# chinajuanbob/istio

Hardware: AMD Instinct MI355X
Metric: request x rule predicate evals/sec at 10k rules (higher is better)
Workload: dtype u32; 1 GPU; C2 rules scaled to R=10000, 1048576 requests per GPU (configs[1] family, configs[4] shard); rules=10000, requests_per_gpu=1048576, parallelism=request-sharded dp1

## Files before the change

istio_amd/csrc/kernels.hip:

```cpp
#include <hip/hip_runtime.h>
#include <stdint.h>
#include <type_traits>

#include "../../include/mxp_batch.h"
#include "kargs.h"
#include "pack_args.h"
#include "vm.h"

namespace {

__device__ __forceinline__ uint32_t uni(uint32_t v) { return __builtin_amdgcn_readfirstlane(v); }

typedef __attribute__((address_space(4))) const mxp_kargs ckargs;
__device__ __forceinline__ ckargs& kargs_view() {
    ckargs* p = (ckargs*)__builtin_amdgcn_kernarg_segment_ptr();
    asm volatile("" : "+s"(p));
    return *p;
}

__device__ __forceinline__ uint32_t wave_max(uint32_t v) {
#pragma unroll
    for (int off = 32; off > 0; off >>= 1) v = max(v, (uint32_t)__shfl_xor((int)v, off, 64));
    return __builtin_amdgcn_readfirstlane(v);
}
// ... 997 lines not shown
                }
                if (old == key) break;
                h = (h + 1u) & (cap - 1u);
            }
            lcls[i] = h;
            if (count) atomicAdd(A.vt_cnt + kb + h, lcnt[i]);
        }
        __syncthreads();
        (void)loc;
        __syncthreads();
    }
}

extern "C" __global__ __launch_bounds__(256) void mxp_vtd_final_kernel(mxp_kargs A, mxp_vtd_final_args F) {
    const uint32_t a = blockIdx.y, i = blockIdx.x * 256u + threadIdx.x;
    if (i >= MXP_VTD_CAP) return;
    const uint64_t at = (uint64_t)F.cand[a] * MXP_VTD_CAP + i;
    const unsigned long long key = F.tkey[at];
    if (key == MXP_VT_EMPTY) return;
    const uint32_t cap = A.vt_meta[a * 8u + MXP_VTM_CAP], kb = A.vt_meta[a * 8u + MXP_VTM_KBASE];
    unsigned long long* T = A.vt_keys + kb;
    uint32_t h = mxp_hash64(key) & (cap - 1u);
    while (atomicCAS(T + h, (unsigned long long)MXP_VT_EMPTY, key) != MXP_VT_EMPTY) h = (h + 1u) & (cap - 1u);
    const uint2 cr = F.tcr[at];
    A.vt_rep[kb + h] = cr.y;
    A.vt_cnt[kb + h] = cr.x;
}

extern "C" hipError_t mxp_launch_vtd_final(const mxp_kargs* args, const mxp_vtd_final_args* f, hipStream_t s) {
    hipLaunchKernelGGL(mxp_vtd_final_kernel, dim3(MXP_VTD_CAP / 256u, args->n_vt), dim3(256), 0, s, *args, *f);
    return hipGetLastError();
}

__device__ __forceinline__ uint32_t vt_probe(const unsigned long long* __restrict__ T, uint32_t cap,
                                             unsigned long long key) {
    uint32_t h = mxp_hash64(key) & (cap - 1u);
    for (uint32_t i = 0; i < cap; i++, h = (h + 1u) & (cap - 1u)) {
        const unsigned long long k = T[h];
        if (k == key || k == MXP_VT_EMPTY) break;
    }
    return h;
}
extern "C" __global__ __launch_bounds__(256) void mxp_vt_lookup_kernel(mxp_kargs A) {
    const uint32_t a = blockIdx.y, q = A.q0 + (blockIdx.x * 256u + threadIdx.x) * 4u, Q1 = A.q1;
    if (q >= Q1) return;
    const uint64_t N = A.n;
    const uint32_t col = uni(A.vt_meta[a * 8u + MXP_VTM_COL]), cap = uni(A.vt_meta[a * 8u + MXP_VTM_CAP]),
                   kb = uni(A.vt_meta[a * 8u + MXP_VTM_KBASE]);
    const unsigned long long* __restrict__ T = A.vt_keys + kb;
    const uint64_t at = (uint64_t)col * N + q;
    uint16_t* const C = A.vt_cls + (uint64_t)a * MXP_VT_PITCH(N) + q;
    if ((N & 3u) == 0 && (q & 3u) == 0 && q + 4u <= Q1) {
        const uint32_t k4 = *(const uint32_t*)(A.kinds + at);
        const ulonglong2 v01 = *(const ulonglong2*)(A.vals + at), v23 = *(const ulonglong2*)(A.vals + at + 2u);
        const uint32_t h0 = vt_probe(T, cap, mxp_vt_key(k4 & 0xFFu, v01.x));
        const uint32_t h1 = vt_probe(T, cap, mxp_vt_key((k4 >> 8) & 0xFFu, v01.y));
        const uint32_t h2 = vt_probe(T, cap, mxp_vt_key((k4 >> 16) & 0xFFu, v23.x));
        const uint32_t h3 = vt_probe(T, cap, mxp_vt_key(k4 >> 24, v23.y));
        *(uint64_t*)C = (uint64_t)h0 | (uint64_t)h1 << 16 | (uint64_t)h2 << 32 | (uint64_t)h3 << 48;
        return;
    }
    for (uint32_t r = 0; r < 4u && q + r < Q1; r++)
        C[r] = (uint16_t)vt_probe(T, cap, mxp_vt_key(A.kinds[at + r], A.vals[at + r]));
}

template <bool kNfa>
__device__ __forceinline__ void vt_eval_body(const mxp_kargs& A, uint64_t (*regs)[256]) {
    const uint32_t tid = threadIdx.x;
    const uint32_t lane = tid & 63u;
    const uint32_t wave = uni(tid >> 6);
    uint32_t t = blockIdx.x, a = 0;
    for (; a + 1 < A.n_vt; a++) {
        const uint32_t nt = uni(A.vt_meta[a * 8u + MXP_VTM_CAP]) / 64u;
        if (t < nt) break;
        t -= nt;
    }
    const uint32_t* M = A.vt_meta + a * 8u;
    const uint32_t cap = uni(M[MXP_VTM_CAP]), kb = uni(M[MXP_VTM_KBASE]), tb = uni(M[MXP_VTM_TBASE]),
                   nw = uni(M[MXP_VTM_NW]), woff = uni(M[MXP_VTM_WOFF]);
    const uint32_t j = blockIdx.y * 4u + wave;
    if (j >= nw || t * 64u >= cap) return;
    const uint32_t k = t * 64u + lane;
    const bool live = __hip_atomic_load(A.vt_keys + kb + k, __ATOMIC_RELAXED, __HIP_MEMORY_SCOPE_AGENT) != MXP_VT_EMPTY;
    const uint32_t rep = live ? A.vt_rep[kb + k] : 0u;
    const uint32_t g = uni(A.vt_words[2u * (woff + j)]), mask = uni(A.vt_words[2u * (woff + j) + 1u]);
    uint32_t m = 0, e = 0;
    for (uint32_t bits = mask; bits; bits &= bits - 1u) {
        const uint32_t b = __builtin_ctz(bits);
        const uint32_t rule = g * 32u + b;
        const uint32_t base = uni(A.rule_off[rule]);
        const uint32_t len = uni(A.rule_off[rule + 1]) - base;
        const uint32_t code = run_rule<false, kNfa>(A, ((cuint32*)A.prog) + (uint64_t)base * 4u, len, 0u, live, rule, rep, regs, tid);
        if (live) {
            m |= code == PC_TRUE ? 1u << b : 0u;
            e |= code >= PC_ERROR ? 1u << b : 0u;
        }
    }
    *(uint2*)(A.vt_tm + 2u * ((uint64_t)tb + (uint64_t)j * cap + k)) = make_uint2(m, e);
    if (counting(A)) {
        const uint32_t c = live ? A.vt_cnt[kb + k] : 0u;
        for (uint32_t bits = wave_or(live ? m : 0u); bits; bits &= bits - 1u) {
            const uint32_t bb = __builtin_ctz(bits);
            uint32_t sum = (m >> bb) & 1u ? c : 0u;
#pragma unroll
            for (int off = 32; off > 0; off >>= 1) sum += (uint32_t)__shfl_xor((int)sum, off, 64);
            if (lane == 0 && sum) atomicAdd(A.hits + g * 32u + bb, (unsigned long long)sum);
        }
    }
}

extern "C" __global__ __launch_bounds__(256) void mxp_vt_eval_kernel(mxp_kargs A) {
    __shared__ uint64_t regs[MXP_VM_MAXREG][256];
    vt_eval_body<false>(A, regs);
}

extern "C" __global__ __launch_bounds__(256) void mxp_vt_eval_nfa_kernel(mxp_kargs A) {
    __shared__ uint64_t regs[MXP_VM_MAXREG][256];
    vt_eval_body<true>(A, regs);
}

__device__ __forceinline__ void sort8(uint32_t (&x)[8]) {
#define MXP_CX(a, b)                          \
    {                                         \
        const uint32_t lo = min(x[a], x[b]);  \
        x[b] = max(x[a], x[b]);               \
        x[a] = lo;                            \
    }
    MXP_CX(0, 1) MXP_CX(2, 3) MXP_CX(4, 5) MXP_CX(6, 7) MXP_CX(0, 2) MXP_CX(1, 3) MXP_CX(4, 6) MXP_CX(5, 7)
    MXP_CX(1, 2) MXP_CX(5, 6) MXP_CX(0, 4) MXP_CX(1, 5) MXP_CX(2, 6) MXP_CX(3, 7) MXP_CX(2, 4) MXP_CX(3, 5)
    MXP_CX(1, 2) MXP_CX(3, 4) MXP_CX(5, 6)
#undef MXP_CX
}

__device__ __forceinline__ void dtp_merge(uint32_t x, bool on, uint32_t (&m)[4], uint32_t (&e)[4]) {
    const uint32_t b = on ? 1u << (x & 31u) : 0u, r = (x >> 5) & 3u;
    const uint32_t bm = (x & 128u) ? 0u : b, be = (x & 128u) ? b : 0u;
#pragma unroll
    for (uint32_t k = 0; k < 4; k++) {
        m[k] |= r == k ? bm : 0u;
        e[k] |= r == k ? be : 0u;
    }
}

struct DtpQueue {
    uint32_t q0 = ~0u, q1 = ~0u, q2 = ~0u, q3 = ~0u;
    __device__ __forceinline__ void load(const mxp_kargs& A, uint32_t chunk, uint32_t req0, bool in) {
        if (!A.dtp_slots || !in) return;
        typedef uint32_t v4u __attribute__((ext_vector_type(4)));
        const uint64_t qi = (uint64_t)chunk * MXP_DTP_ROW(A.dtp_tiles) + (req0 >> 2);
        const uint32_t dk = A.dtp_qn[qi];
        const v4u sl = *(const v4u*)(A.dtp_slots + qi * 8u);
        decode(dk, sl);
    }
    __device__ __forceinline__ void load_live(const uint16_t* slots, const uint8_t* qn, uint32_t tiles, uint32_t chunk,
                                              uint32_t req0, bool in) {
        if (!in) return;
        typedef uint32_t v4u __attribute__((ext_vector_type(4)));
        const uint64_t qi = (uint64_t)chunk * MXP_DTP_ROW(tiles) + (req0 >> 2);
        const uint32_t dk = qn[qi];
        if (!dk) return;
        const v4u sl = *(const v4u*)(slots + qi * 8u);
        decode(dk, sl);
    }
    __device__ __forceinline__ uint32_t head_group() const { return (q0 & 0xFFFFu) == 0xFFFFu ? 256u : (q0 >> 8) & 0xFFu; }
    __device__ __forceinline__ bool take(uint32_t g, uint32_t (&m)[4]) {
        bool named = false;
        while (head_group() == g) {
            const uint32_t x = q0 & 0xFFFFu;
            const bool mp = !(x & 128u);
            const uint32_t b = mp ? 1u << (x & 31u) : 0u, r = (x >> 5) & 3u;
#pragma unroll
            for (uint32_t k = 0; k < 4; k++) m[k] |= r == k ? b : 0u;
            named |= mp;
            q0 = __builtin_amdgcn_alignbit(q1, q0, 16);
            q1 = __builtin_amdgcn_alignbit(q2, q1, 16);
            q2 = __builtin_amdgcn_alignbit(q3, q2, 16);
            q3 = q3 >> 16 | 0xFFFF0000u;
        }
        return named;
    }
    template <typename V4>
    __device__ __forceinline__ void decode(uint32_t dk, const V4& sl) {
        if (!dk) return;
        const uint32_t h[4] = {sl.x, sl.y, sl.z, sl.w};
        uint32_t x[8];
#pragma unroll
        for (uint32_t i = 0; i < 8; i++) x[i] = i < dk ? (h[i >> 1] >> (16u * (i & 1u))) & 0xFFFFu : 0xFFFFu;
        sort8(x);
        q0 = x[0] | x[1] << 16;
        q1 = x[2] | x[3] << 16;
        q2 = x[4] | x[5] << 16;
        q3 = x[6] | x[7] << 16;
    }
    __device__ __forceinline__ bool any_err() const { return __ballot(has_err()) != 0; }
    __device__ __forceinline__ bool has_err() const {
        bool h = false;
        const uint32_t w[4] = {q0, q1, q2, q3};
#pragma unroll
        for (int i = 0; i < 8; i++) {
            const uint32_t x = (w[i >> 1] >> (16 * (i & 1))) & 0xFFFFu;
            h |= x != 0xFFFFu && (x & 128u);
        }
        return h;
    }
    template <uint32_t G, bool kErr>
    __device__ __forceinline__ void merge_c(uint32_t (&m)[4], uint32_t (&e)[4]) {
        for (;;) {
            const uint32_t x = q0;
            const bool hit = ((x >> 8) & 0xFFu) == G;
            if (!__ballot(hit)) break;
            const uint32_t b = hit ? 1u << (x & 31u) : 0u, r = (x >> 5) & 3u;
            const uint32_t bm = (kErr && (x & 128u)) ? 0u : b;
#pragma unroll
            for (uint32_t k = 0; k < 4; k++) m[k] |= r == k ? bm : 0u;
            if (kErr) {
                const uint32_t be = (x & 128u) ? b : 0u;
#pragma unroll
                for (uint32_t k = 0; k < 4; k++) e[k] |= r == k ? be : 0u;
            }
            if (hit) {
                q0 = __builtin_amdgcn_alignbit(q1, q0, 16);
                q1 = __builtin_amdgcn_alignbit(q2, q1, 16);
                q2 = __builtin_amdgcn_alignbit(q3, q2, 16);
                q3 = q3 >> 16 | 0xFFFF0000u;
            }
        }
    }
    __device__ __forceinline__ void merge(uint32_t g, uint32_t (&m)[4], uint32_t (&e)[4]) {
        for (;;) {
            const uint32_t x = q0 & 0xFFFFu;
            const bool hit = (x >> 8) == g;
            if (!__ballot(hit)) break;
            dtp_merge(x, hit, m, e);
            if (hit) {
                q0 = __builtin_amdgcn_alignbit(q1, q0, 16);
                q1 = __builtin_amdgcn_alignbit(q2, q1, 16);
                q2 = __builtin_amdgcn_alignbit(q3, q2, 16);
                q3 = q3 >> 16 | 0xFFFF0000u;
            }
        }
    }
};

template <bool kLds>
__device__ __forceinline__ void vtfill_wave(const mxp_kargs& A, const mxp_fill* F, uint32_t chunk, uint32_t qw,
                                            const uint2* S, const uint32_t* RW) {
    const uint32_t lane = threadIdx.x & 63u;
    const uint32_t col = uni(F->col), okset = uni(F->okset), g0 = uni(F->g0), n = uni(F->n), moff = uni(F->moff);
    const uint64_t N = A.n;
    const uint32_t Q1 = A.q1;
    if (qw >= Q1) return;
    const uint32_t q0 = qw + lane * 4u;
    const bool vec = (N & 3u) == 0 && (Q1 & 3u) == 0 && (q0 & 3u) == 0;
    const uint32_t nvt = uni(A.n_vt);
    uint32_t bad[4];
    typedef uint32_t vcls __attribute__((ext_vector_type(2 * MXP_VT_MAX)));
    vcls clv;
#pragma unroll
    for (int r = 0; r < 4; r++) {
        const bool in = q0 + r < Q1;
        const uint32_t k = in ? A.kinds[(uint64_t)col * N + q0 + r] : 0u;
        bad[r] = (in && !((okset >> k) & 1u)) ? ~0u : 0u;
    }
#pragma unroll
    for (uint32_t a = 0; a < MXP_VT_MAX; a++) {
        uint64_t c = 0;
        if (a < nvt) {
            const uint16_t* C = A.vt_cls + (uint64_t)a * MXP_VT_PITCH(N);
            if (vec && q0 < Q1) {
                c = *(const uint64_t*)(C + q0);
            } else {
                for (uint32_t r = 0; r < 4; r++)
                    if (q0 + r < Q1) c |= (uint64_t)C[q0 + r] << (16u * r);
            }
        }
        clv[2 * a] = (uint32_t)c;
        clv[2 * a + 1] = (uint32_t)(c >> 32);
    }
    const bool any = (bad[0] | bad[1] | bad[2] | bad[3]) != 0;
    DtpQueue dq;
    dq.load(A, chunk, q0, q0 < Q1);
    const bool dany = __ballot(dq.q0 != ~0u) != 0;
    const bool nt = !(A.flags & 128u);
    typedef uint32_t v4u __attribute__((ext_vector_type(4)));
    const uint32_t MV = lane < 2u * MXP_VT_MAX && (lane >> 1) < nvt ? A.vt_meta[(lane >> 1) * 8u + MXP_VTM_CAP + (lane & 1u)] : 0u;
    const uint32_t FM = lane < n ? A.fill_masks[moff + lane] : 0u;
    const uint32_t GM = kLds && lane < n ? A.gvt_mask[g0 + lane] : 0u;
    const uint32_t GO = lane <= n ? A.gvt_off[g0 + lane] : 0u;
    const uint32_t e0 = __builtin_amdgcn_readlane(GO, 0), ecount = __builtin_amdgcn_readlane(GO, n) - e0;
    uint32_t GE0 = lane < ecount ? A.gvt[e0 + lane] : 0u, GE1 = lane + 64u < ecount ? A.gvt[e0 + 64u + lane] : 0u;
    uint32_t anyerr[4] = {0u, 0u, 0u, 0u};
    for (uint32_t g = 0; g < n; g++) {
        const uint32_t G = g0 + g;
        const uint32_t mask = __builtin_amdgcn_readlane(FM, g);
        uint32_t m[4] = {0u, 0u, 0u, 0u}, e[4], ve[4] = {0u, 0u, 0u, 0u};
#pragma unroll
        for (int r = 0; r < 4; r++) e[r] = bad[r] & mask;
        if (A.errlog && any && mask)
            for (uint32_t r = 0; r < 4; r++)
                if (e[r] && q0 + r < Q1) log_guard_errors(A, e[r], G * 32u, q0 + r);
        const uint32_t i0 = __builtin_amdgcn_readlane(GO, g) - e0, i1 = __builtin_amdgcn_readlane(GO, g + 1) - e0;
        if constexpr (kLds) {
            const uint32_t gm = __builtin_amdgcn_readlane(GM, g);
            const uint4 ra = *(const uint4*)(RW + g * MXP_VT_MAX), rb = *(const uint4*)(RW + g * MXP_VT_MAX + 4u);
            const uint32_t rows[MXP_VT_MAX] = {ra.x, ra.y, ra.z, ra.w, rb.x, rb.y, rb.z, rb.w};
#pragma unroll
            for (uint32_t a = 0; a < MXP_VT_MAX; a++) {
                if (!(gm & (1u << a))) continue;
                const uint32_t row = rows[a];
                const uint64_t c = (uint64_t)clv[2u * a] | (uint64_t)clv[2u * a + 1u] << 32;
#pragma unroll
                for (uint32_t r = 0; r < 4; r++) {
                    const uint2 w = S[row + ((uint32_t)(c >> (16u * r)) & 0xFFFFu)];
                    m[r] |= w.x;
                    ve[r] |= w.y;
                }
            }
        } else
        for (uint32_t i = i0; i < i1; i++) {
            const uint32_t ent = i < 64u ? __builtin_amdgcn_readlane(GE0, i)
                                 : i < 128u ? __builtin_amdgcn_readlane(GE1, i - 64u) : uni(A.gvt[e0 + i]);
            const uint32_t a = ent >> 24, j = ent & 0xFFFFFFu;
            const uint32_t au = __builtin_amdgcn_readfirstlane(a);
            const uint64_t c = (uint64_t)clv[2u * au] | (uint64_t)clv[2u * au + 1u] << 32;
            if constexpr (kLds) {
                const uint32_t row = j;
#pragma unroll
                for (uint32_t r = 0; r < 4; r++) {
                    const uint2 w = S[row + ((uint32_t)(c >> (16u * r)) & 0xFFFFu)];
                    m[r] |= w.x;
                    ve[r] |= w.y;
                }
            } else {
                const uint32_t cap = __builtin_amdgcn_readlane(MV, 2u * a);
                const uint32_t tb = __builtin_amdgcn_readlane(MV, 2u * a + 1u);
                const uint64_t row = (uint64_t)tb + (uint64_t)j * cap;
#pragma unroll
                for (uint32_t r = 0; r < 4; r++) {
                    const uint2 w = *(const uint2*)(A.vt_tm + 2u * (row + ((c >> (16u * r)) & 0xFFFFu)));
                    m[r] |= w.x;
                    ve[r] |= w.y;
                }
            }
        }
        uint32_t vmask[4];
#pragma unroll
        for (int r = 0; r < 4; r++) {
            vmask[r] = q0 + r < Q1 ? ~0u : 0u;
            e[r] |= ve[r];
        }
        if (A.errlog) {
            uint32_t c = 0;
#pragma unroll
            for (int r = 0; r < 4; r++) c += (uint32_t)__builtin_popcount(ve[r] & vmask[r]);
            vt_count_n(A, c);
        }
        if (dany) dq.merge(g, m, e);
#pragma unroll
        for (uint32_t r = 0; r < 4; r++) anyerr[r] |= e[r];
        const uint64_t at = (uint64_t)G * N + q0;
        if (vec && q0 < Q1) {
            const v4u mv = v4u{m[0], m[1], m[2], m[3]};
            const v4u ev = v4u{e[0], e[1], e[2], e[3]};
            if (nt) {
                if (A.out_match) __builtin_nontemporal_store(mv, (v4u*)(A.out_match + at));
                if (A.out_err) __builtin_nontemporal_store(ev, (v4u*)(A.out_err + at));
            } else {
                if (A.out_match) *(v4u*)(A.out_match + at) = mv;
                if (A.out_err) *(v4u*)(A.out_err + at) = ev;
            }
        } else {
            for (uint32_t r = 0; r < 4; r++) {
                if (q0 + r >= Q1) break;
                if (A.out_match) A.out_match[at + r] = m[r];
                if (A.out_err) A.out_err[at + r] = e[r];
            }
        }
    }
    if (A.req_err)
        for (uint32_t r = 0; r < 4; r++)
            if (anyerr[r] && q0 + r < Q1) A.req_err[q0 + r] = 1;
}

extern "C" __global__ __launch_bounds__(256) void mxp_fill_dtp_kernel(mxp_kargs A) {
    const uint32_t lane = threadIdx.x & 63u;
    const uint32_t wave = uni(threadIdx.x >> 6);
    const mxp_fill* F = A.fills + blockIdx.y;
    const uint32_t col = uni(F->col), okset = uni(F->okset), g0 = uni(F->g0), n = uni(F->n), moff = uni(F->moff);
    const uint64_t N = A.n;
    const uint32_t Q1 = A.q1;
    const uint32_t qw = A.q0 + (blockIdx.x * 4u + wave) * 256u;
    if (qw >= Q1) return;
    const uint32_t q0 = qw + lane * 4u;
    const bool vec = (N & 3u) == 0 && (Q1 & 3u) == 0;
    uint32_t bad[4];
#pragma unroll
    for (int r = 0; r < 4; r++) {
        const bool in = q0 + r < Q1;
        const uint32_t k = in ? A.kinds[(uint64_t)col * N + q0 + r] : 0u;
        bad[r] = (in && !((okset >> k) & 1u)) ? ~0u : 0u;
    }
    const bool any = (bad[0] | bad[1] | bad[2] | bad[3]) != 0;
    const bool store = !A.dtp_lazy || uni(*A.dtp_lazy) != 0u;
    const bool sparse = A.ret_w && uni(A.ret_w[0]) == 0u;
    DtpQueue dq, dp;
    if (sparse) {
        dq.load_live(A.dtp_slots, A.dtp_qn, A.dtp_tiles, A.dtp_cbase + blockIdx.y, q0, q0 < Q1);
        dp.load_live(A.dtp_pslots, A.dtp_pqn, A.dtp_tiles, A.dtp_cbase + blockIdx.y, q0, q0 < Q1);
    } else if (store) {
        dq.load(A, A.dtp_cbase + blockIdx.y, q0, q0 < Q1);
    }
    const bool dany = __ballot(dq.q0 != ~0u) != 0;
    if (A.req_err && any) {
        uint32_t masks = 0;
        for (uint32_t g = 0; g < n; g++) masks |= uni(A.fill_masks[moff + g]);
        if (masks)
            for (uint32_t r = 0; r < 4; r++)
                if (bad[r] && q0 + r < Q1) A.req_err[q0 + r] = 1;
    }
    if (A.errlog && any)
        for (uint32_t g = 0; g < n; g++) {
            const uint32_t mask = uni(A.fill_masks[moff + g]);
            for (uint32_t r = 0; r < 4; r++)
                if (bad[r] && q0 + r < Q1) log_guard_errors(A, mask, (g0 + g) * 32u, q0 + r);
        }
    if (!store) return;
    const bool nt = !(A.flags & 128u);
    typedef uint32_t v4u __attribute__((ext_vector_type(4)));
    if (sparse) {
        const bool snt = (A.flags & 4194304u) != 0u;
        for (;;) {
            const uint32_t g = min(dq.head_group(), dp.head_group());
            if (g >= n) break;
            uint32_t m[4] = {0u, 0u, 0u, 0u}, z[4] = {0u, 0u, 0u, 0u};
            const bool cur = dq.take(g, m);
            const bool was = dp.take(g, z);
            if (cur || was) {
                const uint64_t at = (uint64_t)(g0 + g) * N + q0;
                if (vec) {
                    const v4u mv = v4u{m[0], m[1], m[2], m[3]};
                    if (snt)
                        __builtin_nontemporal_store(mv, (v4u*)(A.out_match + at));
                    else
                        *(v4u*)(A.out_match + at) = mv;
                } else {
                    for (uint32_t r = 0; r < 4; r++)
                        if (q0 + r < Q1) A.out_match[at + r] = m[r];
                }
            }
        }
        return;
    }
    for (uint32_t g = 0; g < n; g++) {
        const uint32_t mask = uni(A.fill_masks[moff + g]);
        uint32_t m[4] = {0u, 0u, 0u, 0u}, e[4];
#pragma unroll
        for (int r = 0; r < 4; r++) e[r] = bad[r] & mask;
        if (dany) dq.merge(g, m, e);
        const uint64_t at = (uint64_t)(g0 + g) * N + q0;
        if (vec && q0 < Q1) {
            const v4u mv = v4u{m[0], m[1], m[2], m[3]}, ev = v4u{e[0], e[1], e[2], e[3]};
            if (nt) {
                if (A.out_match) __builtin_nontemporal_store(mv, (v4u*)(A.out_match + at));
                if (A.out_err) __builtin_nontemporal_store(ev, (v4u*)(A.out_err + at));
            } else {
                if (A.out_match) *(v4u*)(A.out_match + at) = mv;
                if (A.out_err) *(v4u*)(A.out_err + at) = ev;
            }
        } else {
            for (uint32_t r = 0; r < 4; r++) {
                if (q0 + r >= Q1) break;
                if (A.out_match) A.out_match[at + r] = m[r];
                if (A.out_err) A.out_err[at + r] = e[r];
            }
        }
    }
}

extern "C" __global__ __launch_bounds__(256) void mxp_vtfill_kernel(mxp_kargs A) {
    const uint32_t wave = uni(threadIdx.x >> 6);
    vtfill_wave<false>(A, A.fills + blockIdx.y, A.dtp_cbase + blockIdx.y, A.q0 + (blockIdx.x * 4u + wave) * 256u, nullptr,
                       nullptr);
}

#define MXP_VTF_STAGE 4096u
extern "C" __global__ __launch_bounds__(256) void mxp_vtfill_lds_kernel(mxp_kargs A) {
    __shared__ uint2 S[MXP_VTF_STAGE];
    const uint32_t tid = threadIdx.x, lane = tid & 63u, wave = uni(tid >> 6);
    const mxp_fill* F = A.fills + blockIdx.y;
    const uint32_t g0 = uni(F->g0), n = uni(F->n), nvt = uni(A.n_vt);
    const uint32_t e0 = uni(A.gvt_off[g0]), ecount = uni(A.gvt_off[g0 + n]) - e0;
    const uint32_t E0 = lane < ecount ? A.gvt[e0 + lane] : 0xFFFFFFFFu;
    const uint32_t E1 = lane + 64u < ecount ? A.gvt[e0 + 64u + lane] : 0xFFFFFFFFu;
    const uint32_t capl = lane < nvt ? A.vt_meta[lane * 8u + MXP_VTM_CAP] : 0u;
    const uint32_t tbl = lane < nvt ? A.vt_meta[lane * 8u + MXP_VTM_TBASE] : 0u;
    uint32_t PB = 0, PJ = 0, total = 0;
    for (uint32_t a = 0; a < nvt; a++) {
        const uint32_t lo = wave_min(min((E0 >> 24) == a ? (E0 & 0xFFFFFFu) : 0xFFFFFFFFu,
                                         (E1 >> 24) == a ? (E1 & 0xFFFFFFu) : 0xFFFFFFFFu));
        const uint32_t hi = wave_max(max((E0 >> 24) == a && E0 != 0xFFFFFFFFu ? (E0 & 0xFFFFFFu) + 1u : 0u,
                                         (E1 >> 24) == a && E1 != 0xFFFFFFFFu ? (E1 & 0xFFFFFFu) + 1u : 0u));
        const uint32_t rows = hi > lo ? hi - lo : 0u;
        if (lane == a) {
            PB = total;
            PJ = rows ? lo : 0u;
        }
        total += rows * __builtin_amdgcn_readlane(capl, a);
    }
    const bool staged = ecount <= 128u && n <= MXP_FILL_CHUNK && total <= MXP_VTF_STAGE && !(A.flags & 2097152u);
    __shared__ uint32_t RW[MXP_FILL_CHUNK * MXP_VT_MAX];
    __shared__ uint32_t PL[3 * MXP_VT_MAX];
    if (staged) {
        for (uint32_t a = 0; a < nvt; a++) {
            const uint32_t base = __builtin_amdgcn_readlane(PB, a);
            const uint32_t next = a + 1u < nvt ? __builtin_amdgcn_readlane(PB, a + 1u) : total;
            const uint64_t src = (uint64_t)__builtin_amdgcn_readlane(tbl, a) +
                                 (uint64_t)__builtin_amdgcn_readlane(PJ, a) * __builtin_amdgcn_readlane(capl, a);
            for (uint32_t i = tid; i < next - base; i += 256u) S[base + i] = *(const uint2*)(A.vt_tm + 2u * (src + i));
        }
        if (tid < nvt) {
            PL[3u * tid] = PB;
            PL[3u * tid + 1u] = PJ;
            PL[3u * tid + 2u] = capl;
        }
        __syncthreads();
        if (tid < n) {
            const uint32_t i1 = A.gvt_off[g0 + tid + 1u];
            for (uint32_t i = A.gvt_off[g0 + tid]; i < i1; i++) {
                const uint32_t ent = A.gvt[i], a = ent >> 24, j = ent & 0xFFFFFFu;
                RW[tid * MXP_VT_MAX + a] = PL[3u * a] + (j - PL[3u * a + 1u]) * PL[3u * a + 2u];
            }
        }
        __syncthreads();
    }
    for (uint32_t t = 0; t < MXP_VTF_TILES; t++) {
        const uint32_t qw = A.q0 + ((blockIdx.x * MXP_VTF_TILES + t) * 4u + wave) * 256u;
        if (staged)
            vtfill_wave<true>(A, F, A.dtp_cbase + blockIdx.y, qw, S, RW);
        else
            vtfill_wave<false>(A, F, A.dtp_cbase + blockIdx.y, qw, nullptr, nullptr);
    }
}

#define MXP_VTI_CAP 64u
template <uint32_t V>
struct GroupC {
    static constexpr uint32_t value = V;
    static constexpr bool ct = true;
};
struct GroupR {
    uint32_t value;
    static constexpr bool ct = false;
};
template <uint32_t G, uint32_t NG, typename F>
__device__ __forceinline__ void for_groups(F& f) {
    if constexpr (G < NG) {
        f(GroupC<G>{});
        for_groups<G + 1, NG>(f);
    }
}
template <uint32_t NVT, bool kSlow>
__device__ __forceinline__ void vtfill_imm_body(const mxp_kargs& A, uint32_t bx, uint32_t by, uint32_t gx) {
    __shared__ uint32_t SM[NVT * MXP_FILL_CHUNK * MXP_VTI_CAP];
    __shared__ uint32_t SJ[NVT * MXP_FILL_CHUNK];
    __shared__ uint32_t eflag;
    const uint32_t tid = threadIdx.x, lane = tid & 63u, wave = uni(tid >> 6);
    uint8_t* const slow = A.vtf_slow + ((uint64_t)by * gx + bx) * (MXP_VTF_TILES * 4u);
    if constexpr (kSlow) {
        if (!__syncthreads_or(tid < MXP_VTF_TILES * 4u ? slow[tid] : 0)) return;
    }
    const mxp_fill* F = A.fills + by;
    const uint32_t col = uni(F->col), okset = uni(F->okset), g0 = uni(F->g0), n = uni(F->n), moff = uni(F->moff);
    const uint32_t chunk = A.dtp_cbase + by;
    for (uint32_t i = tid; i < NVT * MXP_FILL_CHUNK * MXP_VTI_CAP; i += 256u) SM[i] = 0u;
    if (tid < NVT * MXP_FILL_CHUNK) SJ[tid] = ~0u;
    if (tid == 0) eflag = 0u;
    __syncthreads();
    const uint32_t TB = lane < NVT ? A.vt_meta[lane * 8u + MXP_VTM_TBASE] : 0u;
    uint32_t eor = 0u;
    for (uint32_t g = 0; g < n; g++) {
        const uint32_t i0 = uni(A.gvt_off[g0 + g]), i1 = uni(A.gvt_off[g0 + g + 1u]);
        for (uint32_t x = tid; x < (i1 - i0) * MXP_VTI_CAP; x += 256u) {
            const uint32_t ent = A.gvt[i0 + x / MXP_VTI_CAP], a = ent >> 24, j = ent & 0xFFFFFFu, k = x % MXP_VTI_CAP;
            const uint32_t tb = __builtin_amdgcn_ds_bpermute((int)(a << 2), (int)TB);
            const uint2 w = *(const uint2*)(A.vt_tm + 2u * ((uint64_t)tb + (uint64_t)j * MXP_VTI_CAP + k));
            SM[(a * MXP_FILL_CHUNK + g) * MXP_VTI_CAP + k] = w.x;
            if (k == 0) SJ[a * MXP_FILL_CHUNK + g] = j;
            eor |= w.y;
        }
    }
    if (__ballot(eor != 0u)) {
        if (lane == 0) atomicOr(&eflag, 1u);
    }
    __syncthreads();
    const bool errs = eflag != 0u;
    const uint64_t N = A.n;
    const uint32_t Q1 = A.q1;
    const bool nt = !(A.flags & 128u);
    typedef uint32_t v4u __attribute__((ext_vector_type(4)));
    const uint32_t FM = lane < n ? A.fill_masks[moff + lane] : 0u;
    struct TileIn {
        uint32_t k4, dk;
        uint64_t c[NVT];
        v4u sl;
    };
    auto fetch = [&](uint32_t t, TileIn& T) __attribute__((always_inline)) {
        const uint32_t q0 = A.q0 + ((bx * MXP_VTF_TILES + t) * 4u + wave) * 256u + lane * 4u;
        const bool vec = (N & 3u) == 0 && (Q1 & 3u) == 0 && (q0 & 3u) == 0;
        T.k4 = 0u;
        if (vec && q0 < Q1) {
            T.k4 = *(const uint32_t*)(A.kinds + (uint64_t)col * N + q0);
        } else {
            for (uint32_t r = 0; r < 4; r++)
                if (q0 + r < Q1) T.k4 |= (uint32_t)A.kinds[(uint64_t)col * N + q0 + r] << (8u * r);
        }
#pragma unroll
        for (uint32_t a = 0; a < NVT; a++) {
            const uint16_t* C = A.vt_cls + (uint64_t)a * MXP_VT_PITCH(N);
            uint64_t c = 0;
            if (vec && q0 < Q1) {
                c = *(const uint64_t*)(C + q0);
            } else {
                for (uint32_t r = 0; r < 4; r++)
                    if (q0 + r < Q1) c |= (uint64_t)C[q0 + r] << (16u * r);
            }
            T.c[a] = c;
        }
        T.dk = 0u;
// ... 896 lines not shown
        if (bits && A.out_match) atomicOr(A.out_match + (uint64_t)w * A.n + req, bits);
        t += (uint32_t)__builtin_popcount(bits);
    }
    if (A.stats) {
#pragma unroll
        for (int off = 32; off > 0; off >>= 1) t += (uint32_t)__shfl_xor((int)t, off, 64);
        if (lane == 0 && t) atomicAdd((unsigned long long*)A.stats, (unsigned long long)t);
    }
}

namespace {

__device__ __forceinline__ void csa(uint32_t& h, uint32_t& l, uint32_t a, uint32_t b, uint32_t c) {
    const uint32_t u = a ^ b;
    h = (a & b) | (u & c);
    l = u ^ c;
}

__device__ __forceinline__ uint32_t hs16(const uint32_t* d, uint32_t& ones, uint32_t& twos, uint32_t& fours,
                                         uint32_t& eights) {
    uint32_t twosA, twosB, foursA, foursB, eightsA, eightsB, sixteens;
    csa(twosA, ones, ones, d[0], d[1]);
    csa(twosB, ones, ones, d[2], d[3]);
    csa(foursA, twos, twos, twosA, twosB);
    csa(twosA, ones, ones, d[4], d[5]);
    csa(twosB, ones, ones, d[6], d[7]);
    csa(foursB, twos, twos, twosA, twosB);
    csa(eightsA, fours, fours, foursA, foursB);
    csa(twosA, ones, ones, d[8], d[9]);
    csa(twosB, ones, ones, d[10], d[11]);
    csa(foursA, twos, twos, twosA, twosB);
    csa(twosA, ones, ones, d[12], d[13]);
    csa(twosB, ones, ones, d[14], d[15]);
    csa(foursB, twos, twos, twosA, twosB);
    csa(eightsB, fours, fours, foursA, foursB);
    csa(sixteens, eights, eights, eightsA, eightsB);
    return sixteens;
}

template <bool kVec>
__device__ __forceinline__ void hits_body(const uint32_t* __restrict__ row, uint32_t n, uint32_t n_rules,
                                          unsigned long long* __restrict__ hits) {
    const uint32_t w = blockIdx.x;
    const uint32_t nthreads = gridDim.y * blockDim.x;
    const uint32_t t = blockIdx.y * blockDim.x + threadIdx.x;
    uint32_t ones = 0, twos = 0, fours = 0, eights = 0, sixteens = 0;
    uint32_t P[8];
#pragma unroll
    for (int j = 0; j < 8; j++) P[j] = 0;
    for (uint64_t base = 0; base < n; base += nthreads * 32u) {
        uint32_t d[32];
        if (kVec) {
#pragma unroll
            for (int j = 0; j < 8; j++) {
                const uint64_t i = base + ((uint64_t)j * nthreads + t) * 4u;
                uint4 v = make_uint4(0, 0, 0, 0);
                if (i < n) v = *(const uint4*)(row + i);
                d[4 * j] = v.x;
                d[4 * j + 1] = v.y;
                d[4 * j + 2] = v.z;
                d[4 * j + 3] = v.w;
            }
        } else {
#pragma unroll
            for (int j = 0; j < 32; j++) {
                const uint64_t i = base + (uint64_t)j * nthreads + t;
                d[j] = i < n ? row[i] : 0u;
            }
        }
        const uint32_t sA = hs16(d, ones, twos, fours, eights);
        const uint32_t sB = hs16(d + 16, ones, twos, fours, eights);
        uint32_t thirtytwos;
        csa(thirtytwos, sixteens, sixteens, sA, sB);
#pragma unroll
        for (int j = 0; j < 8; j++) P[j] += (thirtytwos >> j) & 0x01010101u;
    }
    __shared__ uint32_t red[32][8];
#pragma unroll
    for (int k = 0; k < 32; k++) {
        uint32_t c = 32u * ((P[k & 7] >> (8 * (k >> 3))) & 0xFFu) + 16u * ((sixteens >> k) & 1u) +
                     8u * ((eights >> k) & 1u) + 4u * ((fours >> k) & 1u) + 2u * ((twos >> k) & 1u) + ((ones >> k) & 1u);
        for (int off = 32; off > 0; off >>= 1) c += __shfl_xor((int)c, off, 64);
        if ((threadIdx.x & 63) == 0) red[k][threadIdx.x >> 6] = c;
    }
    __syncthreads();
    if (threadIdx.x < 32) {
        uint32_t c = 0;
        for (uint32_t i = 0; i < blockDim.x / 64; i++) c += red[threadIdx.x][i];
        const uint32_t rule = w * 32 + threadIdx.x;
        if (rule < n_rules && c) atomicAdd(&hits[rule], (unsigned long long)c);
    }
}

}

__device__ __forceinline__ void next_gate(unsigned long long* stats, uint32_t* gate_next, uint32_t n, uint32_t force) {
    if (!gate_next || blockIdx.x || blockIdx.y || threadIdx.x) return;
    const unsigned long long v = *stats;
    *gate_next = force == 1u ? 1u : force == 2u ? 0u : (v * 125ull <= (unsigned long long)gridDim.x * n ? 1u : 0u);
    *stats = 0ull;
}

extern "C" __global__ __launch_bounds__(256) void mxp_hits_kernel(const uint32_t* __restrict__ match, uint32_t n,
                                                                  uint32_t n_rules,
                                                                  unsigned long long* __restrict__ hits,
                                                                  const uint32_t* __restrict__ gate,
                                                                  unsigned long long* stats, uint32_t* gate_next,
                                                                  uint32_t force) {
    next_gate(stats, gate_next, n, force);
    if (gate && *gate) return;
    hits_body<true>(match + (uint64_t)blockIdx.x * n, n, n_rules, hits);
}

extern "C" __global__ __launch_bounds__(256) void mxp_hits_ragged_kernel(const uint32_t* __restrict__ match, uint32_t n,
                                                                         uint32_t n_rules,
                                                                         unsigned long long* __restrict__ hits,
                                                                         const uint32_t* __restrict__ gate,
                                                                         unsigned long long* stats, uint32_t* gate_next,
                                                                         uint32_t force) {
    next_gate(stats, gate_next, n, force);
    if (gate && *gate) return;
    hits_body<false>(match + (uint64_t)blockIdx.x * n, n, n_rules, hits);
}

extern "C" hipError_t mxp_launch_eval(const mxp_kargs* args, uint32_t grid_x, uint32_t grid_y, int vm, hipStream_t s) {
    if (vm == 2 && args->refs)
        hipLaunchKernelGGL(mxp_eval_deep_refs_kernel, dim3(grid_x, grid_y), dim3(256), 0, s, *args);
    else if (vm == 2 && args->nfa)
        hipLaunchKernelGGL(mxp_eval_deep_nfa_kernel, dim3(grid_x, grid_y), dim3(256), 0, s, *args);
    else if (vm == 2)
        hipLaunchKernelGGL(mxp_eval_deep_kernel, dim3(grid_x, grid_y), dim3(256), 0, s, *args);
    else if (vm && args->refs)
        hipLaunchKernelGGL(mxp_eval_refs_kernel, dim3(grid_x, grid_y), dim3(256), 0, s, *args);
    else if (vm && args->nfa)
        hipLaunchKernelGGL(mxp_eval_nfa_kernel, dim3(grid_x, grid_y), dim3(256), 0, s, *args);
    else if (vm)
        hipLaunchKernelGGL(mxp_eval_kernel, dim3(grid_x, grid_y), dim3(256), 0, s, *args);
    else if (args->flags & 65536u)
        hipLaunchKernelGGL(mxp_guard_kernel, dim3(grid_x, grid_y), dim3(256), 0, s, *args);
    else
        hipLaunchKernelGGL(mxp_guard2_kernel, dim3((grid_x + 1) / 2, grid_y), dim3(256), 0, s, *args);
    return hipGetLastError();
}

extern "C" hipError_t mxp_launch_dtp_hits(const uint32_t* part, uint32_t tiles, uint32_t n_rules,
                                          unsigned long long* hits, hipStream_t s) {
    const uint32_t R2 = (n_rules + 1u) / 2u;
    hipLaunchKernelGGL(mxp_dtp_hits_kernel, dim3((R2 + 255u) / 256u, (tiles + 63u) / 64u), dim3(256), 0, s, part, tiles,
                       n_rules, hits);
    return hipGetLastError();
}

extern "C" hipError_t mxp_launch_fill(const mxp_kargs* args, uint32_t n_fills, hipStream_t s) {
    if (args->dtp_slots) {
        hipLaunchKernelGGL(mxp_fill_dtp_kernel, dim3((args->q1 - args->q0 + 1023u) / 1024u, n_fills), dim3(256), 0, s, *args);
        return hipGetLastError();
    }
    const uint32_t per_block = 1024u * (args->fill_span ? args->fill_span : 1u);
    hipLaunchKernelGGL(mxp_fill_kernel, dim3((args->q1 - args->q0 + per_block - 1) / per_block, n_fills), dim3(256), 0, s, *args);
    return hipGetLastError();
}

extern "C" hipError_t mxp_launch_vtfill(const mxp_kargs* args, uint32_t n_fills, hipStream_t s) {
    if (args->flags & 2097152u) {
        hipLaunchKernelGGL(mxp_vtfill_kernel, dim3((args->q1 - args->q0 + 1023u) / 1024u, n_fills), dim3(256), 0, s, *args);
    } else {
        const uint32_t per = 1024u * MXP_VTF_TILES;
        const dim3 grid((args->q1 - args->q0 + per - 1u) / per, n_fills);
        void (*k)(mxp_kargs) = mxp_vtfill_lds_kernel;
        void (*ks)(mxp_kargs, uint32_t, uint32_t) = nullptr;
        if (args->vt_imm && args->vtf_slow && !(args->flags & 33554432u)) {
            switch (args->n_vt) {
#define MXP_VTFILL_CASE(K)                  \
    case K:                                 \
        k = mxp_vtfill_imm##K##_kernel;      \
        ks = mxp_vtfill_imm_slow##K##_kernel; \
        break;
                MXP_VTFILL_CASE(1)
                MXP_VTFILL_CASE(2)
                MXP_VTFILL_CASE(3)
                MXP_VTFILL_CASE(4)
                MXP_VTFILL_CASE(5)
                MXP_VTFILL_CASE(6)
                MXP_VTFILL_CASE(7)
                MXP_VTFILL_CASE(8)
#undef MXP_VTFILL_CASE
            default: break;
            }
        }
        hipLaunchKernelGGL(k, grid, dim3(256), 0, s, *args);
        if (ks) hipLaunchKernelGGL(ks, dim3((grid.x * grid.y + 15u) / 16u), dim3(256), 0, s, *args, grid.x, grid.y);
    }
    return hipGetLastError();
}

extern "C" hipError_t mxp_launch_dtp_sort(const mxp_kargs* args, hipStream_t s) {
    const size_t lds = args->dtp_part ? (size_t)((args->n_rules + 1u) / 2u) * 4u : 0u;
    hipLaunchKernelGGL(mxp_dtp_sort_kernel, dim3(args->dtp_tn ? args->dtp_tn : args->dtp_tiles), dim3(256), lds, s, *args);
    return hipGetLastError();
}

extern "C" hipError_t mxp_launch_vt_classify(const mxp_kargs* args, hipStream_t s) {
    hipLaunchKernelGGL(mxp_vt_classify_kernel, dim3((args->q1 - args->q0 + MXP_VTC_REQ - 1u) / MXP_VTC_REQ), dim3(256), 0, s,
                       *args);
    return hipGetLastError();
}

extern "C" hipError_t mxp_launch_vt_lookup(const mxp_kargs* args, hipStream_t s) {
    hipLaunchKernelGGL(mxp_vt_lookup_kernel, dim3((args->q1 - args->q0 + 1023u) / 1024u, args->n_vt), dim3(256), 0, s, *args);
    return hipGetLastError();
}

extern "C" hipError_t mxp_launch_vt_eval(const mxp_kargs* args, uint32_t tiles, uint32_t wchunks, hipStream_t s) {
    if (!tiles || !wchunks) return hipSuccess;
    if (args->nfa)
        hipLaunchKernelGGL(mxp_vt_eval_nfa_kernel, dim3(tiles, wchunks), dim3(256), 0, s, *args);
    else
        hipLaunchKernelGGL(mxp_vt_eval_kernel, dim3(tiles, wchunks), dim3(256), 0, s, *args);
    return hipGetLastError();
}

extern "C" hipError_t mxp_launch_inject(const mxp_kargs* args, uint32_t grid, hipStream_t s) {
    hipLaunchKernelGGL(mxp_inject_kernel, dim3(grid), dim3(256), 0, s, *args);
    return hipGetLastError();
}

extern "C" hipError_t mxp_launch_index(const mxp_kargs* args, uint32_t grid, hipStream_t s) {
    if (args->refs)
        hipLaunchKernelGGL(mxp_index_refs_kernel, dim3(grid), dim3(256), 0, s, *args);
    else if (args->nfa)
        hipLaunchKernelGGL(mxp_index_nfa_kernel, dim3(grid), dim3(256), 0, s, *args);
    else if (args->dtp_ent && args->wave_t)
        hipLaunchKernelGGL(mxp_index_dtp_prof_kernel, dim3(grid * 4u), dim3(64), 0, s, *args);
    else if (args->dtp_ent && args->tmpl_lite)
        hipLaunchKernelGGL(mxp_index_dtp_lite_kernel, dim3(grid * 4u), dim3(64), 0, s, *args);
    else if (args->dtp_ent)
        hipLaunchKernelGGL(mxp_index_dtp_kernel, dim3(grid * 4u), dim3(64), 0, s, *args);
    else if (args->wave_t)
        hipLaunchKernelGGL(mxp_index_prof_kernel, dim3(grid), dim3(256), 0, s, *args);
    else
        if (args->flags & 8192u)
            hipLaunchKernelGGL(mxp_index5_kernel, dim3(grid), dim3(256), 0, s, *args);
        else
            hipLaunchKernelGGL(mxp_index_kernel, dim3(grid), dim3(256), 0, s, *args);
    return hipGetLastError();
}

extern "C" __global__ __launch_bounds__(256) void mxp_heads_kernel(mxp_kargs A, const uint32_t* __restrict__ cols,
                                                                   uint4* __restrict__ heads) {
    const uint32_t req = blockIdx.x * 256u + threadIdx.x, row = blockIdx.y;
    if (req >= A.n) return;
    const uint64_t at = (uint64_t)cols[row] * A.n + req;
    uint4 h = make_uint4(0u, 0u, 0u, 0u);
    if (A.kinds[at] == MXP_STRING) {
        const StrRef r = str_of(A, A.vals[at]);
        const uint64_t w0 = r.n ? ld8a(r.p) : 0ull, w1 = r.n > 8u ? ld8a(r.p + 8) : 0ull;
        const uint64_t m0 = r.n >= 8u ? ~0ull : (1ull << (r.n * 8u)) - 1ull;
        const uint64_t m1 = r.n >= 12u ? 0xFFFFFFFFull : r.n > 8u ? (1ull << ((r.n - 8u) * 8u)) - 1ull : 0ull;
        h = make_uint4((uint32_t)(w0 & m0), (uint32_t)((w0 & m0) >> 32), (uint32_t)(w1 & m1), r.n);
    }
    heads[(uint64_t)row * A.n + req] = h;
}

extern "C" hipError_t mxp_launch_heads(const mxp_kargs* args, const uint32_t* cols, uint32_t nrow, uint4* heads, hipStream_t s) {
    hipLaunchKernelGGL(mxp_heads_kernel, dim3((args->n + 255u) / 256u, nrow), dim3(256), 0, s, *args, cols, heads);
    return hipGetLastError();
}

extern "C" __global__ void mxp_hits_gate_kernel(const unsigned long long* stats, uint32_t n, uint32_t n_words,
                                                uint32_t* gate, uint32_t force) {
    if (threadIdx.x == 0 && blockIdx.x == 0)
        *gate = force == 1u ? 1u : force == 2u ? 0u : (*stats * 125ull <= (unsigned long long)n_words * n ? 1u : 0u);
}

extern "C" hipError_t mxp_launch_hits_gate(const unsigned long long* stats, uint32_t n, uint32_t n_words,
                                           uint32_t* gate, uint32_t force, hipStream_t s) {
    hipLaunchKernelGGL(mxp_hits_gate_kernel, dim3(1), dim3(64), 0, s, stats, n, n_words, gate, force);
    return hipGetLastError();
}

extern "C" hipError_t mxp_launch_hits(const uint32_t* match, uint32_t n, uint32_t n_rules, uint32_t n_words,
                                      unsigned long long* hits, hipStream_t s, const uint32_t* gate,
                                      unsigned long long* stats, uint32_t* gate_next, uint32_t force) {
    const uint64_t per_block = 256ull * 32u;
    uint64_t gy = (4096u + n_words - 1) / (n_words ? n_words : 1);
    const uint64_t most = (n + per_block - 1) / per_block, least = (n + per_block * 255u - 1) / (per_block * 255u);
    if (gy > most) gy = most;
    if (gy < least) gy = least;
    if (gy < 1) gy = 1;
    if (gy > 65535) return hipErrorInvalidValue;
    if ((n & 3u) == 0 && (((uintptr_t)match) & 15u) == 0)
        hipLaunchKernelGGL(mxp_hits_kernel, dim3(n_words, (uint32_t)gy), dim3(256), 0, s, match, n, n_rules, hits, gate,
                           stats, gate_next, force);
    else
        hipLaunchKernelGGL(mxp_hits_ragged_kernel, dim3(n_words, (uint32_t)gy), dim3(256), 0, s, match, n, n_rules, hits,
                           gate, stats, gate_next, force);
    return hipGetLastError();
}
```

Measured before the change: 59310 billion pairs/s.

## Add tile-major fill kernel that compacts live DTP quads across all fills

Adds mxp_fill_tile_kernel, which runs one block per 1024-request tile and loops over every fill chunk inside it, in place of one block per (tile, fill) pair. In sparse mode it reads the per-quad count bytes for many chunks at once, compacts the non-empty quads into an LDS work queue with ballot/mbcnt, and spreads the decode-and-store work over all threads. Guard-error checking reuses kinds loads when consecutive fills share a column. The aim is to remove the launch and occupancy waste of mostly empty per-fill blocks, at the cost of a more complex kernel with two __syncthreads per chunk batch and new launch preconditions (q0 aligned to 1024, at most 65536 fills).

```diff
diff --git a/istio_amd/csrc/kernels.hip b/istio_amd/csrc/kernels.hip
--- a/istio_amd/csrc/kernels.hip
+++ b/istio_amd/csrc/kernels.hip
@@ -1173,16 +1173,6 @@
         const v4u sl = *(const v4u*)(A.dtp_slots + qi * 8u);
         decode(dk, sl);
     }
-    __device__ __forceinline__ void load_live(const uint16_t* slots, const uint8_t* qn, uint32_t tiles, uint32_t chunk,
-                                              uint32_t req0, bool in) {
-        if (!in) return;
-        typedef uint32_t v4u __attribute__((ext_vector_type(4)));
-        const uint64_t qi = (uint64_t)chunk * MXP_DTP_ROW(tiles) + (req0 >> 2);
-        const uint32_t dk = qn[qi];
-        if (!dk) return;
-        const v4u sl = *(const v4u*)(slots + qi * 8u);
-        decode(dk, sl);
-    }
     __device__ __forceinline__ uint32_t head_group() const { return (q0 & 0xFFFFu) == 0xFFFFu ? 256u : (q0 >> 8) & 0xFFu; }
     __device__ __forceinline__ bool take(uint32_t g, uint32_t (&m)[4]) {
         bool named = false;
@@ -1403,6 +1393,40 @@
             if (anyerr[r] && q0 + r < Q1) A.req_err[q0 + r] = 1;
 }
 
+__device__ __forceinline__ void fill_dtp_groups(const mxp_kargs& A, uint32_t g0, uint32_t n, uint32_t moff,
+                                                const uint32_t (&bad)[4], DtpQueue& dq, uint32_t q0) {
+    const uint64_t N = A.n;
+    const uint32_t Q1 = A.q1;
+    const bool vec = (N & 3u) == 0 && (Q1 & 3u) == 0;
+    const bool dany = __ballot(dq.q0 != ~0u) != 0;
+    const bool nt = !(A.flags & 128u);
+    typedef uint32_t v4u __attribute__((ext_vector_type(4)));
+    for (uint32_t g = 0; g < n; g++) {
+        const uint32_t mask = uni(A.fill_masks[moff + g]);
+        uint32_t m[4] = {0u, 0u, 0u, 0u}, e[4];
+#pragma unroll
+        for (int r = 0; r < 4; r++) e[r] = bad[r] & mask;
+        if (dany) dq.merge(g, m, e);
+        const uint64_t at = (uint64_t)(g0 + g) * N + q0;
+        if (vec && q0 < Q1) {
+            const v4u mv = v4u{m[0], m[1], m[2], m[3]}, ev = v4u{e[0], e[1], e[2], e[3]};
+            if (nt) {
+                if (A.out_match) __builtin_nontemporal_store(mv, (v4u*)(A.out_match + at));
+                if (A.out_err) __builtin_nontemporal_store(ev, (v4u*)(A.out_err + at));
+            } else {
+                if (A.out_match) *(v4u*)(A.out_match + at) = mv;
+                if (A.out_err) *(v4u*)(A.out_err + at) = ev;
+            }
+        } else {
+            for (uint32_t r = 0; r < 4; r++) {
+                if (q0 + r >= Q1) break;
+                if (A.out_match) A.out_match[at + r] = m[r];
+                if (A.out_err) A.out_err[at + r] = e[r];
+            }
+        }
+    }
+}
+
 extern "C" __global__ __launch_bounds__(256) void mxp_fill_dtp_kernel(mxp_kargs A) {
     const uint32_t lane = threadIdx.x & 63u;
     const uint32_t wave = uni(threadIdx.x >> 6);
@@ -1413,7 +1437,6 @@
     const uint32_t qw = A.q0 + (blockIdx.x * 4u + wave) * 256u;
     if (qw >= Q1) return;
     const uint32_t q0 = qw + lane * 4u;
-    const bool vec = (N & 3u) == 0 && (Q1 & 3u) == 0;
     uint32_t bad[4];
 #pragma unroll
     for (int r = 0; r < 4; r++) {
@@ -1423,15 +1446,8 @@
     }
     const bool any = (bad[0] | bad[1] | bad[2] | bad[3]) != 0;
     const bool store = !A.dtp_lazy || uni(*A.dtp_lazy) != 0u;
-    const bool sparse = A.ret_w && uni(A.ret_w[0]) == 0u;
-    DtpQueue dq, dp;
-    if (sparse) {
-        dq.load_live(A.dtp_slots, A.dtp_qn, A.dtp_tiles, A.dtp_cbase + blockIdx.y, q0, q0 < Q1);
-        dp.load_live(A.dtp_pslots, A.dtp_pqn, A.dtp_tiles, A.dtp_cbase + blockIdx.y, q0, q0 < Q1);
-    } else if (store) {
-        dq.load(A, A.dtp_cbase + blockIdx.y, q0, q0 < Q1);
-    }
-    const bool dany = __ballot(dq.q0 != ~0u) != 0;
+    DtpQueue dq;
+    if (store) dq.load(A, A.dtp_cbase + blockIdx.y, q0, q0 < Q1);
     if (A.req_err && any) {
         uint32_t masks = 0;
         for (uint32_t g = 0; g < n; g++) masks |= uni(A.fill_masks[moff + g]);
@@ -1445,11 +1461,34 @@
             for (uint32_t r = 0; r < 4; r++)
                 if (bad[r] && q0 + r < Q1) log_guard_errors(A, mask, (g0 + g) * 32u, q0 + r);
         }
-    if (!store) return;
-    const bool nt = !(A.flags & 128u);
+    if (store) fill_dtp_groups(A, g0, n, moff, bad, dq, q0);
+}
+
+struct FillTileItem {
     typedef uint32_t v4u __attribute__((ext_vector_type(4)));
-    if (sparse) {
+    v4u sc, sp;
+    uint32_t g0, n, dkc = 0u, dkp = 0u, q0;
+    __device__ __forceinline__ void load(const mxp_kargs& A, uint32_t qt, uint32_t e, bool on) {
+        if (!on) return;
+        const uint32_t chunk = e >> 16, quad = (e >> 8) & 0xFFu;
+        dkc = (e >> 4) & 0xFu;
+        dkp = e & 0xFu;
+        q0 = qt + quad * 4u;
+        const uint64_t qi = (uint64_t)(A.dtp_cbase + chunk) * MXP_DTP_ROW(A.dtp_tiles) + (qt >> 2) + quad;
+        if (dkc) sc = *(const v4u*)(A.dtp_slots + qi * 8u);
+        if (dkp) sp = *(const v4u*)(A.dtp_pslots + qi * 8u);
+        g0 = A.fills[chunk].g0;
+        n = A.fills[chunk].n;
+    }
+    __device__ __forceinline__ void finish(const mxp_kargs& A) {
+        const uint64_t N = A.n;
+        const uint32_t Q1 = A.q1;
+        if (!(dkc | dkp) || q0 >= Q1) return;
+        const bool vec = (N & 3u) == 0 && (Q1 & 3u) == 0;
         const bool snt = (A.flags & 4194304u) != 0u;
+        DtpQueue dq, dp;
+        dq.decode(dkc, sc);
+        dp.decode(dkp, sp);
         for (;;) {
             const uint32_t g = min(dq.head_group(), dp.head_group());
             if (g >= n) break;
@@ -1470,31 +1509,117 @@
                 }
             }
         }
-        return;
-    }
-    for (uint32_t g = 0; g < n; g++) {
-        const uint32_t mask = uni(A.fill_masks[moff + g]);
-        uint32_t m[4] = {0u, 0u, 0u, 0u}, e[4];
-#pragma unroll
-        for (int r = 0; r < 4; r++) e[r] = bad[r] & mask;
-        if (dany) dq.merge(g, m, e);
-        const uint64_t at = (uint64_t)(g0 + g) * N + q0;
-        if (vec && q0 < Q1) {
-            const v4u mv = v4u{m[0], m[1], m[2], m[3]}, ev = v4u{e[0], e[1], e[2], e[3]};
-            if (nt) {
-                if (A.out_match) __builtin_nontemporal_store(mv, (v4u*)(A.out_match + at));
-                if (A.out_err) __builtin_nontemporal_store(ev, (v4u*)(A.out_err + at));
-            } else {
-                if (A.out_match) *(v4u*)(A.out_match + at) = mv;
-                if (A.out_err) *(v4u*)(A.out_err + at) = ev;
-            }
-        } else {
-            for (uint32_t r = 0; r < 4; r++) {
-                if (q0 + r >= Q1) break;
-                if (A.out_match) A.out_match[at + r] = m[r];
-                if (A.out_err) A.out_err[at + r] = e[r];
-            }
-        }
+    }
+};
+
+#define MXP_FTQ 8u
+extern "C" __global__ __launch_bounds__(256) void mxp_fill_tile_kernel(mxp_kargs A, uint32_t n_fills) {
+    const uint32_t tid = threadIdx.x, lane = tid & 63u, wave = uni(tid >> 6);
+    const uint64_t N = A.n;
+    const uint32_t Q1 = A.q1;
+    const uint32_t qt = A.q0 + blockIdx.x * 1024u;
+    if (qt >= Q1) return;
+    const uint32_t q0 = qt + tid * 4u;
+    const bool dense = uni(A.ret_w[0]) != 0u;
+    const uint64_t row = MXP_DTP_ROW(A.dtp_tiles);
+    uint32_t cw[MXP_FTQ], pw[MXP_FTQ];
+    auto load_counts = [&](uint32_t c0) {
+#pragma unroll
+        for (uint32_t b = 0; b < MXP_FTQ; b++) {
+            const uint32_t c = min(c0 + wave + 4u * b, n_fills - 1u);
+            const uint64_t at = (uint64_t)(A.dtp_cbase + c) * row + (qt >> 2) + lane * 4u;
+            cw[b] = *(const uint32_t*)(A.dtp_qn + at);
+            pw[b] = *(const uint32_t*)(A.dtp_pqn + at);
+        }
+    };
+    if (!dense) load_counts(0u);
+    {
+        const bool kvec = (N & 3u) == 0 && ((uintptr_t)A.kinds & 3u) == 0;
+        uint32_t col = ~0u, okset = 0u, kb = 0u, bad[4] = {0u, 0u, 0u, 0u}, flagged = 0u;
+        bool any = false;
+        for (uint32_t f0 = 0; f0 < n_fills; f0 += 64u) {
+            const uint32_t fl = min(f0 + lane, n_fills - 1u);
+            const uint32_t colv = A.fills[fl].col, okv = A.fills[fl].okset;
+            const uint32_t f1 = min(64u, n_fills - f0);
+            for (uint32_t i = 0; i < f1; i++) {
+                const uint32_t c = __builtin_amdgcn_readlane(colv, i), ok = __builtin_amdgcn_readlane(okv, i);
+                if (c != col) {
+                    kb = 0u;
+                    if (kvec) {
+                        if (q0 < Q1) kb = *(const uint32_t*)(A.kinds + (uint64_t)c * N + q0);
+                    } else {
+                        for (uint32_t r = 0; r < 4; r++)
+                            if (q0 + r < Q1) kb |= (uint32_t)A.kinds[(uint64_t)c * N + q0 + r] << (8u * r);
+                    }
+                }
+                if (c != col || ok != okset) {
+#pragma unroll
+                    for (uint32_t r = 0; r < 4; r++)
+                        bad[r] = (q0 + r < Q1 && !((ok >> ((kb >> (8u * r)) & 0xFFu)) & 1u)) ? ~0u : 0u;
+                    any = (bad[0] | bad[1] | bad[2] | bad[3]) != 0;
+                }
+                col = c;
+                okset = ok;
+                if (!dense && !__ballot(any)) continue;
+                const mxp_fill* F = A.fills + f0 + i;
+                const uint32_t g0 = uni(F->g0), n = uni(F->n), moff = uni(F->moff);
+                if (A.req_err && any) {
+                    uint32_t masks = 0;
+                    for (uint32_t g = 0; g < n; g++) masks |= uni(A.fill_masks[moff + g]);
+                    if (masks)
+                        for (uint32_t r = 0; r < 4; r++) flagged |= bad[r] & (1u << r);
+                }
+                if (A.errlog && any)
+                    for (uint32_t g = 0; g < n; g++) {
+                        const uint32_t mask = uni(A.fill_masks[moff + g]);
+                        for (uint32_t r = 0; r < 4; r++)
+                            if (bad[r] && q0 + r < Q1) log_guard_errors(A, mask, (g0 + g) * 32u, q0 + r);
+                    }
+                if (dense) {
+                    DtpQueue dq;
+                    dq.load(A, A.dtp_cbase + f0 + i, q0, q0 < Q1);
+                    fill_dtp_groups(A, g0, n, moff, bad, dq, q0);
+                }
+            }
+        }
+        for (uint32_t r = 0; r < 4; r++)
+            if ((flagged >> r) & 1u) A.req_err[q0 + r] = 1;
+    }
+    if (dense) return;
+    __shared__ uint32_t Q[4u][MXP_FTQ * 256u];
+    __shared__ uint32_t Qn[4u];
+    for (uint32_t c0 = 0; c0 < n_fills; c0 += 4u * MXP_FTQ) {
+        if (c0) load_counts(c0);
+        uint32_t run = 0u;
+#pragma unroll
+        for (uint32_t b = 0; b < MXP_FTQ; b++) {
+            const bool in = c0 + wave + 4u * b < n_fills;
+#pragma unroll
+            for (uint32_t k = 0; k < 4u; k++) {
+                const uint32_t dkc = in ? (cw[b] >> (8u * k)) & 0xFFu : 0u, dkp = in ? (pw[b] >> (8u * k)) & 0xFFu : 0u;
+                const bool on = (dkc | dkp) != 0u;
+                const unsigned long long mask = __ballot(on);
+                const uint32_t before =
+                    __builtin_amdgcn_mbcnt_hi((uint32_t)(mask >> 32), __builtin_amdgcn_mbcnt_lo((uint32_t)mask, 0u));
+                if (on) Q[wave][run + before] = (c0 + wave + 4u * b) << 16 | (lane * 4u + k) << 8 | dkc << 4 | dkp;
+                run += (uint32_t)__builtin_popcountll(mask);
+            }
+        }
+        if (lane == 0u) Qn[wave] = run;
+        __syncthreads();
+        const uint32_t t1 = Qn[0], t2 = t1 + Qn[1], t3 = t2 + Qn[2], total = t3 + Qn[3];
+        auto item = [&](uint32_t i) {
+            const uint32_t w = (i >= t1) + (i >= t2) + (i >= t3);
+            return Q[w][i - (w == 0u ? 0u : w == 1u ? t1 : w == 2u ? t2 : t3)];
+        };
+        for (uint32_t i = tid; i < total; i += 512u) {
+            FillTileItem a, b;
+            a.load(A, qt, item(i), true);
+            b.load(A, qt, item(min(i + 256u, total - 1u)), i + 256u < total);
+            a.finish(A);
+            b.finish(A);
+        }
+        __syncthreads();
     }
 }
 
@@ -2697,6 +2822,11 @@
 }
 
 extern "C" hipError_t mxp_launch_fill(const mxp_kargs* args, uint32_t n_fills, hipStream_t s) {
+    if (args->dtp_slots && args->ret_w) {
+        if ((args->q0 & 1023u) || n_fills > 65536u) return hipErrorInvalidValue;
+        hipLaunchKernelGGL(mxp_fill_tile_kernel, dim3((args->q1 - args->q0 + 1023u) / 1024u), dim3(256), 0, s, *args, n_fills);
+        return hipGetLastError();
+    }
     if (args->dtp_slots) {
         hipLaunchKernelGGL(mxp_fill_dtp_kernel, dim3((args->q1 - args->q0 + 1023u) / 1024u, n_fills), dim3(256), 0, s, *args);
         return hipGetLastError();
```

Result: faster. 66290 billion pairs/s (median of 6 runs) (+11.8%).
